# twice154/ofa-for-super-resolution

Hardware: AMD Instinct MI355X
Metric: sr_training_images_per_sec_4x_64to256 (higher is better)
Workload: dtype bf16; 1 GPU; OFA-SR S4 supernet 4x progressive shrinking (elastic kernel {3,5,7}, e=6, d=4, pd=2), LR 64x64 -> HR 256x256, fwd+bwd+Adam, train-mode BN; kernel_transform_mode=1, compat_reference_indexing=True, parallelism=dp1, per_gpu_batch=16, global_batch=16, grad_allreduce_bytes=0, launch=eager

## Files before the change

### include/ofasr.h

```cpp
#ifndef OFASR_H
#define OFASR_H

#include <stddef.h>
#include <stdint.h>

#ifdef __cplusplus
extern "C" {
#endif

#define OFASR_VERSION 303

typedef enum {
    OFASR_OK = 0,
    OFASR_ERR_INVALID_ARG = -1,
    OFASR_ERR_UNSUPPORTED = -2,
    OFASR_ERR_WORKSPACE = -3,
    OFASR_ERR_LAUNCH = -4
} ofasr_status;

typedef enum { OFASR_F32 = 0, OFASR_F16 = 1, OFASR_BF16 = 2 } ofasr_dtype;

int ofasr_version(void);
const char* ofasr_last_error_string(void);
const char* ofasr_status_string(int status);
// ... 151 lines not shown
                               const float* running_var, double eps, int64_t Cin, int64_t Cout, int K, int dtype,
                               void* operands, size_t operand_bytes, void* stream);
int ofasr_conv2d_infer_run(const void* x, void* y, int64_t N, int64_t Cin, int64_t Cout, int64_t H, int64_t W, int K,
                           int dtype, int act, const void* operands, size_t operand_bytes, void* stream);
int ofasr_conv2d_fwd(const void* x, const float* w, void* y, int64_t N, int64_t Cin, int64_t Cout, int64_t H, int64_t W,
                     int K, int dtype, void* workspace, size_t workspace_bytes, void* stream);
int ofasr_conv2d_dgrad(const void* dy, const float* w, void* dx, int64_t N, int64_t Cin, int64_t Cout, int64_t H,
                       int64_t W, int K, int dtype, void* workspace, size_t workspace_bytes, void* stream);
size_t ofasr_conv2d_wgrad_workspace(int64_t N, int64_t Cin, int64_t Cout, int64_t H, int64_t W, int K);
int ofasr_conv2d_wgrad(const void* dy, const void* x, float* dw, int64_t N, int64_t Cin, int64_t Cout, int64_t H,
                       int64_t W, int K, int dtype, void* workspace, size_t workspace_bytes, void* stream);

size_t ofasr_conv2d_f32_workspace(int64_t Cin, int64_t Cout, int K, int dgrad);
int ofasr_conv2d_f32_fwd(const void* x, const float* w, void* y, int64_t N, int64_t Cin, int64_t Cout, int64_t H, int64_t W,
                         int K, void* workspace, size_t workspace_bytes, void* stream);
int ofasr_conv2d_f32_dgrad(const void* dy, const float* w, void* dx, int64_t N, int64_t Cin, int64_t Cout, int64_t H,
                           int64_t W, int K, void* workspace, size_t workspace_bytes, void* stream);
size_t ofasr_conv2d_f32_wgrad_workspace(int64_t N, int64_t Cin, int64_t Cout, int64_t H, int64_t W, int K);
int ofasr_conv2d_f32_wgrad(const void* dy, const void* x, float* dw, int64_t N, int64_t Cin, int64_t Cout, int64_t H,
                           int64_t W, int K, void* workspace, size_t workspace_bytes, void* stream);

size_t ofasr_bicubic_resize_u8_workspace(int64_t planes, int64_t in_h, int64_t in_w, int64_t out_h, int64_t out_w);
int ofasr_bicubic_resize_u8(const void* src, void* dst, int64_t planes, int64_t in_h, int64_t in_w, int64_t out_h,
                            int64_t out_w, void* workspace, size_t workspace_bytes, void* stream);

int ofasr_tile_gather_u8(const void* img, int64_t H, int64_t W, const int64_t* origins, int64_t n, int64_t h, int64_t w,
                         void* out, int dtype, void* stream);
int ofasr_tile_scatter_u8(const void* src, int64_t n, int64_t sh, int64_t sw, int dtype, const int64_t* table, void* img,
                          int64_t OH, int64_t OW, int64_t max_eh, int64_t max_ew, void* stream);

int ofasr_debug_mbfused_tile(int width);
int ofasr_debug_mbfused_split(int enable);
int ofasr_debug_mbconv_bn_bwd_stat(int enable);
long long ofasr_debug_launch_count(const char* substr);
void ofasr_debug_reset_launch_counts(void);
const char* ofasr_debug_launch_table(void);
int ofasr_profile_enable(int on);
const char* ofasr_profile_read(void);

#ifdef __cplusplus
}
#endif
#endif
```

### ofa-for-super-resolution_amd/_C.py

```python
import ctypes
import os
import subprocess

import torch

_HERE = os.path.dirname(os.path.abspath(__file__))
LIB_PATH = os.environ.get("OFASR_LIB_PATH") or os.path.join(_HERE, "csrc", "libofasr_hip.so")

F32, F16, BF16 = 0, 1, 2

_lib = None

_c_i64 = ctypes.c_int64
_c_int = ctypes.c_int
_c_vp = ctypes.c_void_p
_c_sz = ctypes.c_size_t

SIGNATURES = {
    "ofasr_version": (_c_int, []),
    "ofasr_last_error_string": (ctypes.c_char_p, []),
    "ofasr_status_string": (ctypes.c_char_p, [_c_int]),
    "ofasr_pixel_shuffle": (_c_int, [_c_vp, _c_vp, _c_i64, _c_i64, _c_i64, _c_i64, _c_int, _c_int, _c_vp]),
    "ofasr_pixel_unshuffle": (_c_int, [_c_vp, _c_vp, _c_i64, _c_i64, _c_i64, _c_i64, _c_int, _c_int, _c_vp]),
    "ofasr_ktransform_fwd": (_c_int, [_c_vp, ctypes.POINTER(_c_int), _c_int, ctypes.POINTER(_c_vp), _c_int,
# ... 57 lines not shown
    "ofasr_mbconv_stat_floats": (_c_sz, [_c_vp]),
    "ofasr_mbconv_fwd": (_c_int, [_c_vp, _c_vp, _c_vp, _c_vp, _c_vp, _c_sz, _c_vp]),
    "ofasr_mbconv_bwd": (_c_int, [_c_vp, _c_vp, _c_vp, _c_vp, _c_vp, _c_vp, _c_vp, _c_vp, _c_vp, _c_sz, _c_vp]),
    "ofasr_mbstack_fwd": (_c_int, [_c_vp, _c_int, _c_vp, _c_vp]),
    "ofasr_mbstack_bwd": (_c_int, [_c_vp, _c_int, _c_vp, _c_vp, _c_vp]),
    "ofasr_mbconv_defer_join": (_c_int, [_c_int]),
    "ofasr_mbconv_join": (_c_int, [_c_vp]),
    "ofasr_side_stream": (_c_vp, []),
    "ofasr_bicubic_resize_u8_workspace": (_c_sz, [_c_i64, _c_i64, _c_i64, _c_i64, _c_i64]),
    "ofasr_bicubic_resize_u8": (_c_int, [_c_vp, _c_vp, _c_i64, _c_i64, _c_i64, _c_i64, _c_i64, _c_vp, _c_sz, _c_vp]),
    "ofasr_mbconv_infer_supported": (_c_int, [_c_vp]),
    "ofasr_mbconv_infer_workspace": (_c_sz, [_c_vp]),
    "ofasr_mbconv_infer": (_c_int, [_c_vp, _c_vp, _c_vp, _c_vp, _c_sz, _c_vp]),
    "ofasr_mbconv_infer_operand_bytes": (_c_sz, [_c_vp]),
    "ofasr_mbconv_infer_scratch_bytes": (_c_sz, [_c_vp]),
    "ofasr_mbconv_infer_prepare": (_c_int, [_c_vp, _c_vp, _c_sz, _c_vp]),
    "ofasr_mbconv_infer_run": (_c_int, [_c_vp, _c_vp, _c_vp, _c_vp, _c_sz, _c_vp, _c_sz, _c_vp]),
    "ofasr_mbconv_infer_f32_supported": (_c_int, [_c_vp]),
    "ofasr_mbconv_infer_f32_operand_bytes": (_c_sz, [_c_vp]),
    "ofasr_mbconv_infer_f32_scratch_bytes": (_c_sz, [_c_vp]),
    "ofasr_mbconv_infer_f32_prepare": (_c_int, [_c_vp, _c_vp, _c_sz, _c_vp]),
    "ofasr_mbconv_infer_f32_run": (_c_int, [_c_vp, _c_vp, _c_vp, _c_vp, _c_sz, _c_vp, _c_sz, _c_vp]),
    "ofasr_mbconv_recal_f32_supported": (_c_int, [_c_vp]),
    "ofasr_mbconv_recal_f32_workspace": (_c_sz, [_c_vp]),
    "ofasr_mbconv_recal_f32": (_c_int, [_c_vp, _c_vp, _c_vp, _c_vp, _c_vp, _c_vp, _c_vp, _c_sz, _c_vp]),
    "ofasr_bn_recal_accumulate": (_c_int, [_c_vp, _c_i64, _c_i64, ctypes.c_double, ctypes.c_double, _c_vp, _c_vp,
                                           ctypes.c_double, _c_vp, _c_vp, _c_vp]),
    "ofasr_tile_gather_u8": (_c_int, [_c_vp, _c_i64, _c_i64, _c_vp, _c_i64, _c_i64, _c_i64, _c_vp, _c_int, _c_vp]),
    "ofasr_tile_scatter_u8": (_c_int, [_c_vp, _c_i64, _c_i64, _c_i64, _c_int, _c_vp, _c_vp, _c_i64, _c_i64, _c_i64, _c_i64,
                                       _c_vp]),
    "ofasr_debug_mbfused_tile": (_c_int, [_c_int]),
    "ofasr_debug_mbfused_split": (_c_int, [_c_int]),
    "ofasr_debug_mbconv_bn_bwd_stat": (_c_int, [_c_int]),
    "ofasr_debug_launch_count": (ctypes.c_longlong, [ctypes.c_char_p]),
    "ofasr_debug_reset_launch_counts": (None, []),
    "ofasr_debug_launch_table": (ctypes.c_char_p, []),
    "ofasr_profile_enable": (_c_int, [_c_int]),
    "ofasr_profile_read": (ctypes.c_char_p, []),
}


def launch_count(substr=""):
    return int(lib().ofasr_debug_launch_count(substr.encode()))


def reset_launch_counts():
    lib().ofasr_debug_reset_launch_counts()


def launch_table():
    out = {}
    for line in lib().ofasr_debug_launch_table().decode().splitlines():
        n, name = line.split("\t", 1)
        if int(n):
            out[name] = int(n)
    return out


def profile_read():
    out = {}
    for line in lib().ofasr_profile_read().decode().splitlines():
        name, n, us, by, fl = line.rsplit("\t", 4)
        out[name] = {"launches": float(n), "total_us": float(us), "bytes": float(by), "flops": float(fl)}
    return out


# ... 57 lines not shown
```

### ofa-for-super-resolution_amd/csrc/mbconv.hip

```cpp
#include "ofasr_common.h"

#include <atomic>
#include <mutex>
#include <vector>

namespace ofasr {

static size_t align_up(size_t v, size_t a) { return (v + a - 1) / a * a; }
static bool bn_fold_enabled() {
    static const bool on = [] { const char* e = getenv("OFASR_MBCONV_BN_BWD_FOLD"); return !(e && e[0] == '0'); }();
    return on;
}
static thread_local int t_skip_kt = 0;
static std::atomic<int> g_bn_bwd_stat{[] { const char* e = getenv("OFASR_MBCONV_BN_BWD_STAT"); return (e && e[0] == '1') ? 1 : 0; }()};

struct MbSizes {
    size_t es;
    size_t mid_elems;
    size_t out_elems;
    size_t ws_bn;
    size_t ws_bn_bwd;
    size_t ws_dw;
    size_t ws_pw;
    size_t ws_kt;
    size_t scratch;
    size_t stat_a;
    size_t side;
    size_t df_bytes;
    size_t coef_off;
    size_t total;
};

static MbSizes mb_sizes(const ofasr_mbconv_desc* d) {
    MbSizes s;
    const int64_t HW = d->H * d->W;
    s.es = d->dtype == OFASR_F32 ? 4 : 2;
    s.mid_elems = (size_t)(d->N * d->mid * HW);
    s.out_elems = (size_t)(d->N * d->Cout * HW);
    const int64_t cbig = d->mid > d->Cout ? d->mid : d->Cout;
    s.ws_bn = align_up(ofasr_bn_workspace(d->N, cbig), 256);
    s.ws_bn_bwd = align_up(ofasr_bn_act_bwd_workspace(d->N, cbig), 256);
    s.ws_dw = align_up(ofasr_dwconv_wgrad_workspace(d->N, d->mid, d->H, d->W, d->K), 256);
    size_t pw1 = ofasr_pwconv_wgrad_workspace(d->N, d->Cin, d->mid, HW);
    size_t pw2 = ofasr_pwconv_wgrad_workspace(d->N, d->mid, d->Cout, HW);
    s.ws_pw = align_up(pw1 > pw2 ? pw1 : pw2, 256);
    s.ws_kt = align_up(ofasr_ktransform_bwd_workspace(d->ks, d->chain_len - 1, d->mid), 256);
    s.scratch = s.ws_bn > s.ws_bn_bwd ? s.ws_bn : s.ws_bn_bwd;
    {
        const size_t u1 = (size_t)pwconv_stat_units(d->N, d->Cin, HW) * (size_t)d->mid;
        const size_t u2 = (size_t)dwconv_stat_units(d->N, d->H, d->W, d->K, d->dtype) * (size_t)d->mid;
        const size_t u3 = (size_t)pwconv_stat_units(d->N, d->mid, HW) * (size_t)d->Cout;
        s.stat_a = align_up((u1 > u3 ? u1 : u3) * sizeof(float2), 256);
        const size_t ws_stat = s.stat_a + align_up(u2 * sizeof(float2), 256);
        if (ws_stat > s.scratch) s.scratch = ws_stat;
    }
    s.side = s.ws_dw > s.ws_pw ? s.ws_dw : s.ws_pw;
    s.df_bytes = align_up((size_t)(d->mid * d->K * d->K) * sizeof(float), 256);
    s.coef_off = s.scratch + s.side + s.df_bytes + s.ws_kt + 256;
    s.total = s.coef_off + align_up((size_t)(4 * d->mid) * sizeof(float), 256);
    return s;
}

static int check_desc(const char* name, const ofasr_mbconv_desc* d) {
    OFASR_REQUIRE(d != nullptr, OFASR_ERR_INVALID_ARG, "%s: null descriptor", name);
    OFASR_REQUIRE(d->N > 0 && d->Cin > 0 && d->mid > 0 && d->Cout > 0 && d->H > 0 && d->W > 0, OFASR_ERR_INVALID_ARG,
                  "%s: bad shape", name);
    OFASR_REQUIRE(d->chain_len >= 1 && d->chain_len <= 4, OFASR_ERR_INVALID_ARG, "%s: bad kernel chain", name);
    OFASR_REQUIRE(d->ks[d->chain_len - 1] == d->K, OFASR_ERR_INVALID_ARG, "%s: chain does not end at K", name);
    OFASR_REQUIRE(d->w1 && d->w2 && d->wdw_max, OFASR_ERR_INVALID_ARG, "%s: null weight", name);
    OFASR_REQUIRE(!d->residual || d->Cin == d->Cout, OFASR_ERR_INVALID_ARG, "%s: residual needs Cin == Cout", name);
    for (int i = 0; i < 3; ++i)
        OFASR_REQUIRE(d->gamma[i] && d->beta[i] && d->running_mean[i] && d->running_var[i], OFASR_ERR_INVALID_ARG,
                      "%s: null BN tensor %d", name, i);
    return OFASR_OK;
}

__global__ void bump_counters_kernel(int64_t* a, int64_t* b, int64_t* c) {
    if (threadIdx.x == 0) {
        if (a) *a += 1;
        if (b) *b += 1;
        if (c) *c += 1;
    }
}

struct PendingSide {
    const char *t0, *t1, *w0, *w1;
    hipEvent_t done;
};
constexpr size_t MAX_PENDING = 64;
struct SideStream {
    bool ready = false, enabled = true, defer = false;
    hipStream_t s = nullptr;
// ... 375 lines not shown
        if (e1 == hipSuccess) e1 = hipStreamWaitEvent(ss.s, ss.fork[i], 0);
        OFASR_REQUIRE(e1 == hipSuccess, OFASR_ERR_LAUNCH, "%s: stream fork failed: %s", name, hipGetErrorString(e1));
        return OFASR_OK;
    };
    const bool fused = lay.fused;
    if (fused)
        OFASR_REQUIRE((reinterpret_cast<uintptr_t>(tmp_buf) & 15) == 0, OFASR_ERR_UNSUPPORTED,
                      "%s: tmp_buf must be 16-byte aligned (the forward pass did not materialise the activations)", name);
    rc = fork(0);
    if (rc) return rc;
    if (split_fill && !prezeroed) {
        const hipError_t ef = fill(0, 3, (hipStream_t)sst);
        OFASR_REQUIRE(ef == hipSuccess, OFASR_ERR_LAUNCH, "%s: memset failed: %s", name, hipGetErrorString(ef));
    }
    if (fused)
        rc = pwconv_wgrad_xf(t3, y2, g->dw2, d->ldw2, d->N, d->mid, d->Cout, HW, d->dtype,
                             xf_of(stat_buf, 1, d->mid, d->Cout), side_ws, s.side, sst);
    else
        rc = ofasr_pwconv_wgrad(t3, a2, g->dw2, d->ldw2, d->N, d->mid, d->Cout, HW, d->dtype, side_ws, s.side, sst);
    if (rc) return rc;
    StatView s2 = stat_view(sb, 1, d->mid, d->Cout);
    StatView s1 = stat_view(sb, 0, d->mid, d->Cout);
    const bool bn_fold = bn_fold_enabled();
    float* coef = reinterpret_cast<float*>((char*)workspace + s.coef_off);
    void* tC = t + (2 * s.mid_elems + (size_t)d->N * d->Cout * HW) * s.es;
    const bool wg_bx = fused && bn_fold_enabled() &&
                       dwconv_wgrad_bx_supported(tA, y1, y2, d->N, d->mid, d->H, d->W, d->K, d->dtype);
    BwdXf bx2{y2, s2.mean, s2.scale, s2.shift, coef, coef + d->mid, wg_bx ? nullptr : tC};
    static const bool wg1_env = [] { const char* e = getenv("OFASR_MBCONV_WG1_BX"); return e && e[0] == '1'; }();
    const bool wg1_bx = fused && bn_fold && wg1_env &&
                        pwconv_wgrad_bx_supported(tB, y1, x, d->Cin, d->mid, HW, d->dtype);
    BwdXf bx1{y1, s1.mean, s1.scale, s1.shift, coef + 2 * d->mid, coef + 3 * d->mid,
              wg1_bx ? nullptr : (wg_bx ? tC : tA)};
    static const bool coef_fold = [] { const char* e = getenv("OFASR_MBCONV_BN_COEF_FOLD"); return !(e && e[0] == '0'); }();
    auto arm_fold = [&](BwdXf& bx, int P, const StatView& sv, int which) {
        bx.fold_partial = (const double*)workspace;
        bx.fold_P = P;
        bx.fold_C = (int)d->mid;
        bx.fold_training = d->bn_training[which];
        bx.fold_M = (double)d->N * (double)HW;
        bx.fold_invstd = sv.invstd;
        bx.fold_dgamma = g->dgamma[which];
        bx.fold_dbeta = g->dbeta[which];
        bx.coef_ka = const_cast<float*>(bx.ka);
        bx.coef_kbi = const_cast<float*>(bx.kbi);
    };
    const bool bxp = fused && bn_fold && dwconv_xf_supported(tA, tB, d->H, d->W, d->K, d->dtype) &&
                     (reinterpret_cast<uintptr_t>(tC) & 15) == 0 &&
                     pwconv_dgrad_bx_supported(tB, y1, dx, d->residual ? dout : nullptr, d->w1, d->ldw1, d->Cin, d->mid, HW,
                                               d->dtype);
    const bool bn_stat = g_bn_bwd_stat.load(std::memory_order_relaxed) != 0;
    const int P2b = pwconv_stat_units(d->N, d->Cout, HW);
    const bool st2 = bxp && bn_stat && pwconv_dgrad_bstat_supported(t3, y2, tA, d->w2, d->ldw2, d->mid, d->Cout, HW, d->dtype) &&
                     (size_t)P2b * (size_t)d->mid * sizeof(float2) <= s.stat_a;
    if (st2) {
        rc = pwconv_dgrad_bstat(t3, d->w2, d->ldw2, tA, d->N, d->mid, d->Cout, HW, d->dtype,
                                BwdStatOut{y2, s2.mean, s2.scale, s2.shift, (float2*)workspace, P2b}, stream);
        if (rc) return rc;
        rc = bn_bwd_coef_cp((const float2*)workspace, P2b, d->mid, (double)d->N * (double)HW, d->bn_training[1], s2.scale,
                            s2.invstd, g->dgamma[1], g->dbeta[1], coef, coef + d->mid, stream);
    } else {
        rc = ofasr_pwconv_dgrad(t3, d->w2, d->ldw2, tA, d->N, d->mid, d->Cout, HW, d->dtype, stream);
    }
    if (rc) return rc;
    if (bxp) {
        if (!st2 && coef_fold) {
// ... 5 lines not shown
        } else if (!st2) {
            rc = bn_bwd_reduce_coef(tA, y2, s2.scale, s2.shift, s2.mean, s2.invstd, g->dgamma[1], g->dbeta[1], coef,
                                    coef + d->mid, d->N, d->mid, HW, 1, d->bn_training[1], d->dtype, workspace, s.scratch,
                                    stream);
            if (rc) return rc;
        }
        rc = dwconv_dgrad_bx(tA, f, tB, d->N, d->mid, d->H, d->W, d->K, d->dtype, bx2, stream);
        if (rc) return rc;
        rc = fork(1);
        if (rc) return rc;
        if (wg_bx)
            rc = dwconv_wgrad_xf_bx(tA, y1, dfp, d->N, d->mid, d->H, d->W, d->K, d->dtype, xf_of(stat_buf, 0, d->mid, d->Cout),
                                    BwdXf{y2, s2.mean, s2.scale, s2.shift, coef, coef + d->mid, nullptr}, sst);
        else
            rc = dwconv_wgrad_xf(tC, y1, dfp, d->N, d->mid, d->H, d->W, d->K, d->dtype, xf_of(stat_buf, 0, d->mid, d->Cout),
                                 side_ws, s.side, sst);
        if (rc) return rc;
        rc = (t_skip_kt & 2) ? OFASR_OK
                             : ofasr_ktransform_bwd(d->wdw_max, d->ks, d->chain_len - 1, d->mats, d->transform, dfp, g->dwdw_max,
                                                    g->dmats, d->mid, kt_ws, s.ws_kt + 256, sst);
        if (rc) return rc;
        if (coef_fold) {
            int P1 = 0;
            rc = bn_bwd_reduce_only(tB, y1, s1.scale, s1.shift, s1.mean, s1.invstd, d->N, d->mid, HW, 1, d->dtype, workspace,
                                    s.scratch, &P1, stream);
            if (rc) return rc;
            arm_fold(bx1, P1, s1, 0);
        } else {
            rc = bn_bwd_reduce_coef(tB, y1, s1.scale, s1.shift, s1.mean, s1.invstd, g->dgamma[0], g->dbeta[0], coef + 2 * d->mid,
                                    coef + 3 * d->mid, d->N, d->mid, HW, 1, d->bn_training[0], d->dtype, workspace, s.scratch,
                                    stream);
        }
        if (rc) return rc;
        rc = pwconv_dgrad_add_bx(tB, d->w1, d->ldw1, dx, d->residual ? dout : nullptr, d->N, d->Cin, d->mid, HW, d->dtype, bx1,
                                 stream);
        if (rc) return rc;
        rc = fork(2);
        if (rc) return rc;
        if (wg1_bx)
            rc = pwconv_wgrad_bx(tB, x, g->dw1, d->ldw1, d->N, d->Cin, d->mid, HW, d->dtype,
                                 BwdXf{y1, s1.mean, s1.scale, s1.shift, coef + 2 * d->mid, coef + 3 * d->mid, nullptr}, side_ws,
                                 s.side, sst);
        else
            rc = ofasr_pwconv_wgrad(wg_bx ? tC : tA, x, g->dw1, d->ldw1, d->N, d->Cin, d->mid, HW, d->dtype, side_ws, s.side, sst);
        if (rc) return rc;
    } else {
    rc = ofasr_bn_act_bwd(tA, y2, nullptr, tA, nullptr, s2.scale, s2.shift, s2.mean, s2.invstd, g->dgamma[1],
                          g->dbeta[1], d->N, d->mid, HW, 1, d->bn_training[1], d->dtype, workspace, s.scratch, stream);
    if (rc) return rc;
    rc = fork(1);
    if (rc) return rc;
    if (fused)
        rc = dwconv_wgrad_xf(tA, y1, dfp, d->N, d->mid, d->H, d->W, d->K, d->dtype, xf_of(stat_buf, 0, d->mid, d->Cout),
                             side_ws, s.side, sst);
    else
        rc = ofasr_dwconv_wgrad(tA, a1, dfp, d->N, d->mid, d->H, d->W, d->K, d->dtype, side_ws, s.side, sst);
    if (rc) return rc;
    rc = (t_skip_kt & 2) ? OFASR_OK
                         : ofasr_ktransform_bwd(d->wdw_max, d->ks, d->chain_len - 1, d->mats, d->transform, dfp, g->dwdw_max,
                                                g->dmats, d->mid, kt_ws, s.ws_kt + 256, sst);
    if (rc) return rc;
    rc = ofasr_dwconv_dgrad(tA, f, tB, d->N, d->mid, d->H, d->W, d->K, d->dtype, stream);
    if (rc) return rc;
    rc = ofasr_bn_act_bwd(tB, y1, nullptr, tB, nullptr, s1.scale, s1.shift, s1.mean, s1.invstd, g->dgamma[0],
                          g->dbeta[0], d->N, d->mid, HW, 1, d->bn_training[0], d->dtype, workspace, s.scratch, stream);
    if (rc) return rc;
    rc = fork(2);
    if (rc) return rc;
    rc = ofasr_pwconv_wgrad(tB, x, g->dw1, d->ldw1, d->N, d->Cin, d->mid, HW, d->dtype, side_ws, s.side, sst);
    if (rc) return rc;
    if (d->residual)
        rc = pwconv_dgrad_add(tB, d->w1, d->ldw1, dx, dout, d->N, d->Cin, d->mid, HW, d->dtype, stream);
    else
        rc = ofasr_pwconv_dgrad(tB, d->w1, d->ldw1, dx, d->N, d->Cin, d->mid, HW, d->dtype, stream);
    if (rc) return rc;
    }
    if (par) {
        std::lock_guard<std::mutex> lk(ss.mu);
// ... 139 lines not shown
                hipEvent_t ev = nullptr;
                if (hipEventCreateWithFlags(&ev, hipEventDisableTiming) != hipSuccess) {
                    (void)hipGetLastError();
                    return join_side_locked(ss, as_stream(stream), "ofasr_mbstack_bwd");
                }
                ss.pool.push_back(ev);
            }
            const hipError_t e3 = hipEventRecord(ss.pool[k], ss.s);
            OFASR_REQUIRE(e3 == hipSuccess, OFASR_ERR_LAUNCH, "ofasr_mbstack_bwd: event record failed: %s", hipGetErrorString(e3));
            const char *wlo = nullptr, *whi = nullptr;
            for (int i = 0; i < n; ++i) {
                const char* w0 = (const char*)items[i].workspace;
                wlo = (!wlo || w0 < wlo) ? w0 : wlo;
                whi = (!whi || w0 + items[i].workspace_bytes > whi) ? w0 + items[i].workspace_bytes : whi;
            }
            ss.pending.push_back(PendingSide{nullptr, nullptr, wlo, whi, ss.pool[k]});
        } else {
            rc = join_side_locked(ss, as_stream(stream), "ofasr_mbstack_bwd");
        }
    }
    return rc;
}

OFASR_EXPORT int ofasr_mbconv_bwd(const ofasr_mbconv_desc* d, const void* x, const void* act_buf, const float* stat_buf,
                                  const void* dout, void* dx, void* tmp_buf, const ofasr_mbconv_grads* g,
                                  void* workspace, size_t workspace_bytes, void* stream) {
    return mbconv_bwd_impl(d, x, act_buf, stat_buf, dout, dx, tmp_buf, g, workspace, workspace_bytes, stream, false);
}

OFASR_EXPORT int ofasr_debug_mbconv_bn_bwd_stat(int enable) {
    return g_bn_bwd_stat.exchange(enable ? 1 : 0, std::memory_order_relaxed);
}

OFASR_EXPORT int ofasr_mbconv_defer_join(int enable) {
    SideStream& ss = side_stream();
    std::lock_guard<std::mutex> lk(ss.mu);
    const int was = ss.defer ? 1 : 0;
    if (!enable && ss.defer && !ss.pending.empty()) {
        (void)hipStreamSynchronize(ss.s);
        ss.pending.clear();
    }
    ss.defer = ss.enabled && enable != 0;
    return was;
}

OFASR_EXPORT void* ofasr_side_stream(void) {
    SideStream& ss = side_stream();
    return ss.enabled ? (void*)ss.s : nullptr;
}

OFASR_EXPORT int ofasr_mbconv_join(void* stream) {
    SideStream& ss = side_stream();
    std::lock_guard<std::mutex> lk(ss.mu);
    if (ss.pending.empty()) return OFASR_OK;
    return join_side_locked(ss, as_stream(stream), "ofasr_mbconv_join");
}
```

### ofa-for-super-resolution_amd/csrc/ofasr_common.h

```cpp
#pragma once
#include <hip/hip_runtime.h>
#include <hip/hip_ext.h>
#include <tuple>
#include <utility>
#include <stdint.h>
#include <stdio.h>
#include "../../include/ofasr.h"

#define OFASR_EXPORT extern "C" __attribute__((visibility("default")))

namespace ofasr {

void set_error(const char* fmt, ...);

inline hipStream_t as_stream(void* s) { return reinterpret_cast<hipStream_t>(s); }

inline int check_launch(const char* what) {
    hipError_t e = hipGetLastError();
    if (e != hipSuccess) {
        set_error("%s: launch failed: %s", what, hipGetErrorString(e));
        return OFASR_ERR_LAUNCH;
    }
    return OFASR_OK;
}
// ... 288 lines not shown
bool conv_thin_wgrad_supported(int64_t Ct, int64_t Cw, int K, int64_t H, int64_t W, int dtype, const void* a, const void* b);
size_t conv_thin_wgrad_workspace(int64_t N, int64_t Ct, int64_t Cw, int64_t H, int64_t W, int K, int dtype);
int conv_thin_wgrad(const void* dy, const void* x, float* dw, int64_t N, int64_t Cin, int64_t Cout, int64_t H, int64_t W, int K,
                    int dtype, void* workspace, size_t workspace_bytes, void* stream);
bool conv_thin_in_supported(int64_t Ct, int64_t Cw, int K, int64_t W, int dtype, const void* x, const void* y);
int conv_thin_in_units(int64_t N, int64_t Ct, int64_t Cw, int64_t H, int64_t W, int dtype);
int conv_thin_in(const void* x, const float* w, void* y, int64_t N, int64_t Ct, int64_t Cw, int64_t H, int64_t W, int K,
                 int dtype, int dgrad, StatOut so, void* stream);

bool dwconv_xf_supported(const void* x, const void* y, int64_t H, int64_t W, int K, int dtype);
bool dwconv_stat_supported(const void* x, const void* y, int64_t H, int64_t W, int K, int dtype);
int dwconv_fwd_stat(const void* x, const float* f, void* y, int64_t N, int64_t C, int64_t H, int64_t W, int K, int dtype,
                    StatOut so, void* stream);
int dwconv_fwd_xf(const void* x, const float* f, void* y, int64_t N, int64_t C, int64_t H, int64_t W, int K, int dtype,
                  InputXf xf, void* stream, StatOut so = StatOut{nullptr, 0}, BnFold fold = BnFold{});
int dwconv_wgrad_xf(const void* dy, const void* x, float* df, int64_t N, int64_t C, int64_t H, int64_t W, int K,
                    int dtype, InputXf xf, void* workspace, size_t workspace_bytes, void* stream);
bool dwconv_wgrad_bx_supported(const void* da, const void* x, const void* y, int64_t N, int64_t C, int64_t H, int64_t W,
                               int K, int dtype);
int dwconv_wgrad_xf_bx(const void* da, const void* x, float* df, int64_t N, int64_t C, int64_t H, int64_t W, int K,
                       int dtype, InputXf xf, BwdXf bx, void* stream);
int dwconv_dgrad_bx(const void* da, const float* f, void* dx, int64_t N, int64_t C, int64_t H, int64_t W, int K,
                    int dtype, BwdXf bx, void* stream);
int bn_finalize_bump(const void* workspace, int64_t n_partials, int64_t C, double count, const float* gamma,
                     const float* beta, float* running_mean, float* running_var, double momentum, double eps,
                     int training, float* mean, float* invstd, float* scale, float* shift, int64_t* k0, int64_t* k1,
                     int64_t* k2, void* stream);
int pwconv_dgrad_add(const void* dy, const float* w, int64_t ldw, void* dx, const void* addend, int64_t N, int64_t Cin,
                     int64_t Cout, int64_t HW, int dtype, void* stream);
bool pwconv_dgrad_bx_supported(const void* da, const void* y, const void* dx, const void* addend, const float* w,
                               int64_t ldw, int64_t Cin, int64_t Cout, int64_t HW, int dtype);
int pwconv_dgrad_add_bx(const void* da, const float* w, int64_t ldw, void* dx, const void* addend, int64_t N, int64_t Cin,
                        int64_t Cout, int64_t HW, int dtype, BwdXf bx, void* stream);
bool pwconv_xf_supported(const void* x, const void* y, int64_t HW, int dtype);
int pwconv_fwd_xf(const void* x, const float* w, int64_t ldw, void* y, int64_t N, int64_t Cin, int64_t Cout, int64_t HW,
                  int dtype, InputXf xf, void* stream, StatOut so = StatOut{nullptr, 0});
bool pwconv_fold_supported(const void* x, const void* y, const float* w, int64_t ldw, int64_t Cin, int64_t HW, int dtype);
int pwconv_fwd_fold(const void* x, const float* w, int64_t ldw, void* y, int64_t N, int64_t Cin, int64_t Cout,
                    int64_t HW, int dtype, BnFold fold, void* stream, StatOut so = StatOut{nullptr, 0});
int pwconv_fwd_stat(const void* x, const float* w, int64_t ldw, void* y, int64_t N, int64_t Cin, int64_t Cout,
                    int64_t HW, int dtype, StatOut so, void* stream);
bool pwconv_wgrad_bx_supported(const void* da, const void* y, const void* x, int64_t Cin, int64_t Cout, int64_t HW, int dtype);
int pwconv_wgrad_bx(const void* da, const void* x, float* dw, int64_t ldw, int64_t N, int64_t Cin, int64_t Cout, int64_t HW,
                    int dtype, BwdXf bx, void* workspace, size_t workspace_bytes, void* stream);
int pwconv_wgrad_xf(const void* dy, const void* x, float* dw, int64_t ldw, int64_t N, int64_t Cin, int64_t Cout,
                    int64_t HW, int dtype, InputXf xf, void* workspace, size_t workspace_bytes, void* stream);

}
```

### ofa-for-super-resolution_amd/csrc/pwconv.hip

```cpp
#include <stdlib.h>
#include "ofasr_common.h"

namespace ofasr {

typedef __attribute__((ext_vector_type(16))) float f32x16;
typedef __attribute__((ext_vector_type(8))) __bf16 bf16x8;
typedef __attribute__((ext_vector_type(8))) _Float16 f16x8;
typedef __attribute__((ext_vector_type(4))) short s16x4;
typedef __attribute__((ext_vector_type(8))) short s16x8;
typedef __attribute__((address_space(3))) s16x4 lds_s16x4;

constexpr int PW_THREADS = 256;
constexpr int PW_TILE = 128;
constexpr int XROW16 = 320;
constexpr int XROW32 = 512;
constexpr int WROW16 = 128;
constexpr int WROW32 = 256;

template <typename T> struct Mma16;
template <> struct Mma16<bf16_t> {
    static __device__ __forceinline__ f32x16 run(s16x8 a, s16x8 b, f32x16 c) {
        return __builtin_amdgcn_mfma_f32_32x32x16_bf16(__builtin_bit_cast(bf16x8, a), __builtin_bit_cast(bf16x8, b),
                                                       c, 0, 0, 0);
    }
// ... 1092 lines not shown
        T* yw = yn + (long long)(32 * cb) * HW + px;
        if (addend) {
            const T* aw = addend + ((long long)n * wv.M + m_base + 32 * cb) * HW + px;
            uint32_t ar[16];
#pragma unroll
            for (int reg = 0; reg < 16; ++reg)
                ar[reg] = *reinterpret_cast<const uint32_t*>(aw + (long long)acc_row(reg, h) * HW);
#pragma unroll
            for (int reg = 0; reg < 16; ++reg) {
                T lo, hi;
                lo.v = (uint16_t)(ar[reg] & 0xffffu);
                hi.v = (uint16_t)(ar[reg] >> 16);
                acc[0][reg] += to_float(lo);
                acc[1][reg] += to_float(hi);
            }
        }
#pragma unroll
        for (int reg = 0; reg < 16; ++reg)
            *reinterpret_cast<uint32_t*>(yw + (long long)acc_row(reg, h) * HW) = pack2<T>(acc[0][reg], acc[1][reg]);
        if (so.partial) stat_epilogue<T, 2>(acc, px, HW, c, h, 32 * cb, mloc, m_base, so, 2 * tile + hh);
        return;
    }
#pragma unroll
    for (int reg = 0; reg < 16; ++reg) {
        const int r = 32 * cb + acc_row(reg, h);
        if (r < mloc) {
            float v[2] = {acc[0][reg], acc[1][reg]};
            if (addend)
                add_px<T, 2, true>(addend + ((long long)n * wv.M + m_base + r) * HW, p0 + 64 * hh + 2 * c, HW, v);
            store_px<T, 2, true>(yn + (long long)r * HW, p0 + 64 * hh + 2 * c, HW, v);
        }
    }
    if (so.partial) stat_epilogue<T, 2>(acc, p0 + 64 * hh + 2 * c, HW, c, h, 32 * cb, mloc, m_base, so, 2 * tile + hh);
}

template <typename T, bool ALIGNED>
__device__ __forceinline__ void stage_rows64(char* Lt, const T* __restrict__ base, int rows_total, int r0, int HW,
                                             int p0) {
    const int tid = threadIdx.x;
    if constexpr (Elem<T>::is16) {
        if (ALIGNED) {
#pragma unroll
            for (int it = 0; it < 2; ++it) {
                const int q = tid + it * PW_THREADS;
                const int r = q >> 3, ch = q & 7;
                const int px = p0 + 8 * ch;
                uint4 v = make_uint4(0, 0, 0, 0);
                if (r0 + r < rows_total && px < HW)
                    v = *reinterpret_cast<const uint4*>(base + (long long)(r0 + r) * HW + px);
                *reinterpret_cast<uint4*>(Lt + wtile_chunk_off<T>(r, ch)) = v;
            }
        } else {
            for (int e = tid; e < 64 * 64; e += PW_THREADS) {
                const int r = e >> 6, k = e & 63;
                uint16_t v = 0;
                if (r0 + r < rows_total && p0 + k < HW)
                    v = reinterpret_cast<const uint16_t*>(base)[(long long)(r0 + r) * HW + p0 + k];
                *reinterpret_cast<uint16_t*>(Lt + wtile_off<T>(r, k)) = v;
            }
        }
    } else {
        if (ALIGNED) {
#pragma unroll
            for (int it = 0; it < 4; ++it) {
                const int q = tid + it * PW_THREADS;
                const int r = q >> 4, ch = q & 15;
// ... 640 lines not shown
template <typename T>
static int launch_dgrad_bx(const char* name, const void* da, WView wv, void* dx, const void* addend, int64_t N, int64_t HW,
                           BwdXf bx, hipStream_t st) {
    const int tiles_per_img = (int)cdiv(HW, PW_TILE);
    const int64_t total64 = N * tiles_per_img;
    OFASR_REQUIRE(total64 <= INT32_MAX, OFASR_ERR_UNSUPPORTED, "%s: too many pixel tiles", name);
    {
        const double px = (double)N * (double)HW, es = (double)sizeof(T);
        prof_note(es * px * (2.0 * wv.K + wv.M + (addend ? wv.M : 0)) + 4.0 * wv.K * wv.M, 2.0 * px * wv.K * wv.M);
    }
    dim3 grid((unsigned)total64, (unsigned)cdiv(wv.M, 64));
    OFASR_LAUNCH((pw_fanin_pipe_kernel<T, false, true, true>), grid, dim3(PW_THREADS), 0, st, (const T*)da, wv, (T*)dx,
                 (int)HW, tiles_per_img, (int)cdiv(wv.K, 64), InputXf{}, (const T*)addend, StatOut{nullptr, 0}, BnFold{}, bx);
    return check_launch(name);
}

int pwconv_dgrad_add_bx(const void* da, const float* w, int64_t ldw, void* dx, const void* addend, int64_t N, int64_t Cin,
                        int64_t Cout, int64_t HW, int dtype, BwdXf bx, void* stream) {
    const char* name = "pwconv_dgrad_add_bx";
    int rc = check_pw_args(name, da, w, dx, ldw, N, Cin, Cout, HW, dtype);
    if (rc) return rc;
    OFASR_REQUIRE(bx.y && bx.mean && bx.scale && bx.shift &&
                      ((bx.ka && bx.kbi) || (bx.fold_partial && bx.fold_invstd && bx.fold_P > 0 && bx.fold_C == Cout)),
                  OFASR_ERR_INVALID_ARG, "%s: null transform", name);
    OFASR_REQUIRE(pwconv_dgrad_bx_supported(da, bx.y, dx, addend, w, ldw, Cin, Cout, HW, dtype), OFASR_ERR_UNSUPPORTED,
                  "%s: needs the pipelined fan-in kernel (aligned 16-bit tensors, 64 < Cout <= %d)", name, FOLD_KMAX);
    if (N * HW == 0) return OFASR_OK;
    WView wv{w, 1, ldw, (int)Cin, (int)Cout};
    hipStream_t st = as_stream(stream);
    if (dtype == OFASR_F16) return launch_dgrad_bx<f16_t>(name, da, wv, dx, addend, N, HW, bx, st);
    return launch_dgrad_bx<bf16_t>(name, da, wv, dx, addend, N, HW, bx, st);
}

bool pwconv_xf_supported(const void* x, const void* y, int64_t HW, int dtype) {
    return (dtype == OFASR_F16 || dtype == OFASR_BF16) && aligned_for(x, y, HW, true);
}

bool pwconv_dgrad_bstat_supported(const void* dy, const void* y, const void* dx, const float* w, int64_t ldw, int64_t Cin,
                                  int64_t Cout, int64_t HW, int dtype) {
    const bool wvec = (reinterpret_cast<uintptr_t>(w) & 15) == 0 && (ldw % 4) == 0;
    return (dtype == OFASR_F16 || dtype == OFASR_BF16) && aligned_for(dy, dx, HW, true) &&
           (reinterpret_cast<uintptr_t>(y) & 15) == 0 && wvec && Cout == 64 && (Cin == 2 * FO_ROWS || Cin == 3 * FO_ROWS) &&
           HW % PW_TILE == 0;
}

template <typename T>
static int launch_dgrad_bstat(const void* dy, WView wv, void* dx, int64_t N, int64_t HW, BwdStatOut bs, hipStream_t st) {
    const int tiles_per_img = (int)(HW / PW_TILE);
    const int total_tiles = (int)(N * tiles_per_img);
    const double px = (double)N * (double)HW;
    prof_note(2.0 * px * (wv.K + 2.0 * wv.M) + 4.0 * wv.K * wv.M, 2.0 * px * wv.K * wv.M);
    if (wv.M == 3 * FO_ROWS)
        OFASR_LAUNCH((pw_fanout_slabs_kernel<T, 3, 2>), dim3((unsigned)total_tiles), dim3(PW_THREADS), 0, st, (const T*)dy, wv,
                     (T*)dx, (int)HW, tiles_per_img, StatOut{nullptr, 0}, bs);
    else
        OFASR_LAUNCH((pw_fanout_slabs_kernel<T, 2, 2>), dim3((unsigned)total_tiles), dim3(PW_THREADS), 0, st, (const T*)dy, wv,
                     (T*)dx, (int)HW, tiles_per_img, StatOut{nullptr, 0}, bs);
    return check_launch("pwconv_dgrad_bstat");
}

int pwconv_dgrad_bstat(const void* dy, const float* w, int64_t ldw, void* dx, int64_t N, int64_t Cin, int64_t Cout,
                       int64_t HW, int dtype, BwdStatOut bs, void* stream) {
    const char* name = "pwconv_dgrad_bstat";
    int rc = check_pw_args(name, dy, w, dx, ldw, N, Cin, Cout, HW, dtype);
    if (rc) return rc;
    OFASR_REQUIRE(bs.y && bs.mean && bs.scale && bs.shift && bs.partial, OFASR_ERR_INVALID_ARG, "%s: null pointer", name);
// ... 160 lines not shown
```

Baseline: 2713 images/s.

## Fuse expand-conv weight gradient into the BN-backward dgrad fan-in kernel

Adds a kernel that, while computing the first pointwise conv's input gradient with the BN backward transform applied on load, also accumulates the weight gradient from the same transformed tiles against the block input, writing per-block fp32 slabs. A separate reduction then sums the slabs into dw1 on the side stream. This removes the separate wgrad pass that re-read the transformed gradient and input from memory. In exchange it adds shared-memory pressure, slab workspace and an extra reduction launch. It is enabled by default when the shape allows and there are at least 256 pixel-pair tiles.

```diff
diff --git a/include/ofasr.h b/include/ofasr.h
--- a/include/ofasr.h
+++ b/include/ofasr.h
@@ -207,6 +207,7 @@
 int ofasr_debug_mbfused_tile(int width);
 int ofasr_debug_mbfused_split(int enable);
 int ofasr_debug_mbconv_bn_bwd_stat(int enable);
+int ofasr_debug_mbconv_wg1_fused(int enable);
 long long ofasr_debug_launch_count(const char* substr);
 void ofasr_debug_reset_launch_counts(void);
 const char* ofasr_debug_launch_table(void);
diff --git a/ofa-for-super-resolution_amd/_C.py b/ofa-for-super-resolution_amd/_C.py
--- a/ofa-for-super-resolution_amd/_C.py
+++ b/ofa-for-super-resolution_amd/_C.py
@@ -113,6 +113,7 @@
     "ofasr_debug_mbfused_tile": (_c_int, [_c_int]),
     "ofasr_debug_mbfused_split": (_c_int, [_c_int]),
     "ofasr_debug_mbconv_bn_bwd_stat": (_c_int, [_c_int]),
+    "ofasr_debug_mbconv_wg1_fused": (_c_int, [_c_int]),
     "ofasr_debug_launch_count": (ctypes.c_longlong, [ctypes.c_char_p]),
     "ofasr_debug_reset_launch_counts": (None, []),
     "ofasr_debug_launch_table": (ctypes.c_char_p, []),
diff --git a/ofa-for-super-resolution_amd/csrc/mbconv.hip b/ofa-for-super-resolution_amd/csrc/mbconv.hip
--- a/ofa-for-super-resolution_amd/csrc/mbconv.hip
+++ b/ofa-for-super-resolution_amd/csrc/mbconv.hip
@@ -13,6 +13,7 @@
 }
 static thread_local int t_skip_kt = 0;
 static std::atomic<int> g_bn_bwd_stat{[] { const char* e = getenv("OFASR_MBCONV_BN_BWD_STAT"); return (e && e[0] == '1') ? 1 : 0; }()};
+static std::atomic<int> g_wg1_fused{[] { const char* e = getenv("OFASR_MBCONV_WG1_FUSED"); return (e && (e[0] == '0' || e[0] == '1')) ? e[0] - '0' : -1; }()};
 
 struct MbSizes {
     size_t es;
@@ -28,6 +29,8 @@
     size_t side;
     size_t df_bytes;
     size_t coef_off;
+    size_t wg1_off;
+    size_t wg1_bytes;
     size_t total;
 };
 
@@ -57,7 +60,10 @@
     s.side = s.ws_dw > s.ws_pw ? s.ws_dw : s.ws_pw;
     s.df_bytes = align_up((size_t)(d->mid * d->K * d->K) * sizeof(float), 256);
     s.coef_off = s.scratch + s.side + s.df_bytes + s.ws_kt + 256;
-    s.total = s.coef_off + align_up((size_t)(4 * d->mid) * sizeof(float), 256);
+    s.wg1_off = s.coef_off + align_up((size_t)(4 * d->mid) * sizeof(float), 256);
+    const bool wg1_shape = d->dtype != OFASR_F32 && d->Cin == 64 && d->mid % 64 == 0 && d->mid > 64 && d->mid <= 384 && HW % 256 == 0;
+    s.wg1_bytes = wg1_shape ? align_up(pwconv_dgrad_bx_wg_workspace(d->N, d->Cin, d->mid, HW), 256) : 0;
+    s.total = s.wg1_off + s.wg1_bytes;
     return s;
 }
 
@@ -499,6 +505,8 @@
                         pwconv_wgrad_bx_supported(tB, y1, x, d->Cin, d->mid, HW, d->dtype);
     BwdXf bx1{y1, s1.mean, s1.scale, s1.shift, coef + 2 * d->mid, coef + 3 * d->mid,
               wg1_bx ? nullptr : (wg_bx ? tC : tA)};
+    const int wg1_sw = g_wg1_fused.load(std::memory_order_relaxed);
+    const bool wg1_fused_on = wg1_sw > 0 || (wg1_sw < 0 && d->N * (HW / 256) >= 256);
     static const bool coef_fold = [] { const char* e = getenv("OFASR_MBCONV_BN_COEF_FOLD"); return !(e && e[0] == '0'); }();
     auto arm_fold = [&](BwdXf& bx, int P, const StatView& sv, int which) {
         bx.fold_partial = (const double*)workspace;
@@ -570,6 +578,21 @@
                                     stream);
         }
         if (rc) return rc;
+        const bool wg1_fused = wg1_fused_on && s.wg1_bytes > 0 &&
+                               pwconv_dgrad_bx_wg_supported(tB, y1, dx, d->residual ? dout : nullptr, d->w1, d->ldw1, x, d->Cin,
+                                                            d->mid, HW, d->dtype);
+        if (wg1_fused) {
+            char* slabs = (char*)workspace + s.wg1_off;
+            int nslabs = 0;
+            bx1.dy_out = nullptr;
+            rc = pwconv_dgrad_add_bx_wg(tB, d->w1, d->ldw1, dx, d->residual ? dout : nullptr, x, d->N, d->Cin, d->mid, HW,
+                                        d->dtype, bx1, slabs, s.wg1_bytes, &nslabs, stream);
+            if (rc) return rc;
+            rc = fork(2);
+            if (rc) return rc;
+            rc = pwconv_wg_slab_reduce(slabs, nslabs, g->dw1, d->ldw1, d->Cin, d->mid, sst);
+            if (rc) return rc;
+        } else {
         rc = pwconv_dgrad_add_bx(tB, d->w1, d->ldw1, dx, d->residual ? dout : nullptr, d->N, d->Cin, d->mid, HW, d->dtype, bx1,
                                  stream);
         if (rc) return rc;
@@ -582,6 +605,7 @@
         else
             rc = ofasr_pwconv_wgrad(wg_bx ? tC : tA, x, g->dw1, d->ldw1, d->N, d->Cin, d->mid, HW, d->dtype, side_ws, s.side, sst);
         if (rc) return rc;
+        }
     } else {
     rc = ofasr_bn_act_bwd(tA, y2, nullptr, tA, nullptr, s2.scale, s2.shift, s2.mean, s2.invstd, g->dgamma[1],
                           g->dbeta[1], d->N, d->mid, HW, 1, d->bn_training[1], d->dtype, workspace, s.scratch, stream);
@@ -787,6 +811,10 @@
     return g_bn_bwd_stat.exchange(enable ? 1 : 0, std::memory_order_relaxed);
 }
 
+OFASR_EXPORT int ofasr_debug_mbconv_wg1_fused(int enable) {
+    return g_wg1_fused.exchange(enable < 0 ? -1 : (enable ? 1 : 0), std::memory_order_relaxed);
+}
+
 OFASR_EXPORT int ofasr_mbconv_defer_join(int enable) {
     SideStream& ss = side_stream();
     std::lock_guard<std::mutex> lk(ss.mu);
diff --git a/ofa-for-super-resolution_amd/csrc/ofasr_common.h b/ofa-for-super-resolution_amd/csrc/ofasr_common.h
--- a/ofa-for-super-resolution_amd/csrc/ofasr_common.h
+++ b/ofa-for-super-resolution_amd/csrc/ofasr_common.h
@@ -344,6 +344,13 @@
                                int64_t ldw, int64_t Cin, int64_t Cout, int64_t HW, int dtype);
 int pwconv_dgrad_add_bx(const void* da, const float* w, int64_t ldw, void* dx, const void* addend, int64_t N, int64_t Cin,
                         int64_t Cout, int64_t HW, int dtype, BwdXf bx, void* stream);
+bool pwconv_dgrad_bx_wg_supported(const void* da, const void* y, const void* dx, const void* addend, const float* w,
+                                  int64_t ldw, const void* x, int64_t Cin, int64_t Cout, int64_t HW, int dtype);
+size_t pwconv_dgrad_bx_wg_workspace(int64_t N, int64_t Cin, int64_t Cout, int64_t HW);
+int pwconv_dgrad_add_bx_wg(const void* da, const float* w, int64_t ldw, void* dx, const void* addend, const void* x,
+                           int64_t N, int64_t Cin, int64_t Cout, int64_t HW, int dtype, BwdXf bx, void* slabs,
+                           size_t slab_bytes, int* nslabs, void* stream);
+int pwconv_wg_slab_reduce(const void* slabs, int nslabs, float* dw, int64_t ldw, int64_t Cin, int64_t Cout, void* stream);
 bool pwconv_xf_supported(const void* x, const void* y, int64_t HW, int dtype);
 int pwconv_fwd_xf(const void* x, const float* w, int64_t ldw, void* y, int64_t N, int64_t Cin, int64_t Cout, int64_t HW,
                   int dtype, InputXf xf, void* stream, StatOut so = StatOut{nullptr, 0});
diff --git a/ofa-for-super-resolution_amd/csrc/pwconv.hip b/ofa-for-super-resolution_amd/csrc/pwconv.hip
--- a/ofa-for-super-resolution_amd/csrc/pwconv.hip
+++ b/ofa-for-super-resolution_amd/csrc/pwconv.hip
@@ -1148,6 +1148,196 @@
         }
     }
     if (so.partial) stat_epilogue<T, 2>(acc, p0 + 64 * hh + 2 * c, HW, c, h, 32 * cb, mloc, m_base, so, 2 * tile + hh);
+}
+
+constexpr int WGF_THREADS = 512;
+constexpr int WGF_XT_ROW = 256;
+__device__ __forceinline__ int wgf_xt_off(int row, int chunk) { return row * WGF_XT_ROW + ((chunk ^ (row & 15)) << 4); }
+
+template <typename T, int KC>
+__global__ void __launch_bounds__(WGF_THREADS) pw_fanin_wg_kernel(const T* __restrict__ da, const float* __restrict__ w,
+                                                                  long long ldw, T* __restrict__ dx,
+                                                                  const T* __restrict__ xin, float* __restrict__ part,
+                                                                  int HW, int pairs_per_img, int npairs,
+                                                                  const T* __restrict__ addend, BwdXf bx) {
+    constexpr int K = 64 * KC;
+    constexpr int M = 64;
+    __shared__ __attribute__((aligned(16))) char Ws[64 * WROW16];
+    __shared__ __attribute__((aligned(16))) char Xs[2][64 * XROW16];
+    __shared__ __attribute__((aligned(16))) char Xn[2][64 * WGF_XT_ROW];
+    __shared__ __attribute__((aligned(16))) char Xt[2][64 * WGF_XT_ROW];
+    __shared__ float bxt[5 * K];
+    const int tid = threadIdx.x;
+    for (int ch = tid; ch < K; ch += WGF_THREADS) {
+        const float mu = bx.mean[ch], sc = bx.scale[ch];
+        bxt[ch] = mu;
+        bxt[K + ch] = sc;
+        bxt[2 * K + ch] = fmaf(mu, sc, bx.shift[ch]);
+        if (bx.fold_partial) {
+            float ka, kbi;
+            bwdxf_fold(bx, ch, sc, blockIdx.x == 0, ka, kbi);
+            bxt[3 * K + ch] = ka;
+            bxt[4 * K + ch] = kbi;
+        } else {
+            bxt[3 * K + ch] = bx.ka[ch];
+            bxt[4 * K + ch] = bx.kbi[ch];
+        }
+    }
+    __syncthreads();
+    const int lane = lane_id();
+    const int wave = __builtin_amdgcn_readfirstlane((int)(threadIdx.x >> 6));
+    const int half = wave >> 2;
+    const int t = tid & 255;
+    const int c = lane & 31, h = lane >> 5;
+    const int cb = wave & 1, hh = (wave >> 1) & 1;
+    char* Xh = Xs[half];
+    uint32_t xoff[4], woff[2];
+#pragma unroll
+    for (int it = 0; it < 4; ++it) {
+        const int q = t + it * 256;
+        xoff[it] = (uint32_t)(q >> 4) * (uint32_t)HW + 8u * (q & 15);
+    }
+#pragma unroll
+    for (int it = 0; it < 2; ++it) {
+        const int q = tid + it * WGF_THREADS;
+        woff[it] = (uint32_t)(q >> 4) * (uint32_t)ldw + 4u * (q & 15);
+    }
+    constexpr int NOWN = (KC + 1) / 2;
+    f32x16 dwa[NOWN];
+#pragma unroll
+    for (int o = 0; o < NOWN; ++o) dwa[o] = zero16();
+    const int row = 32 * cb + c;
+
+    const int pair_lo = (int)((long long)blockIdx.x * npairs / gridDim.x);
+    const int pair_hi = (int)((long long)(blockIdx.x + 1) * npairs / gridDim.x);
+    for (int pair = pair_lo; pair < pair_hi; ++pair) {
+        const int n = pair / pairs_per_img;
+        const int p0 = (pair - n * pairs_per_img) * (2 * PW_TILE) + PW_TILE * half;
+        const T* dan = da + (long long)n * K * HW + p0;
+        const T* y1n = reinterpret_cast<const T*>(bx.y) + (long long)n * K * HW + p0;
+#pragma unroll
+        for (int it = 0; it < 4; ++it) asm volatile("" : "+v"(xoff[it]));
+#pragma unroll
+        for (int it = 0; it < 2; ++it) asm volatile("" : "+v"(woff[it]));
+        uint4 xr[4], yr[4], xt[4];
+        float4 wr[2];
+        auto load_chunk = [&](int kc) {
+#pragma unroll
+            for (int it = 0; it < 4; ++it) asm volatile("" : "+v"(xoff[it]));
+#pragma unroll
+            for (int it = 0; it < 2; ++it) asm volatile("" : "+v"(woff[it]));
+            const float* wk = w + (long long)(64 * kc) * ldw;
+            const T* xk = dan + (long long)(64 * kc) * HW;
+            const T* yk = y1n + (long long)(64 * kc) * HW;
+#pragma unroll
+            for (int it = 0; it < 2; ++it) wr[it] = *reinterpret_cast<const float4*>(wk + woff[it]);
+#pragma unroll
+            for (int it = 0; it < 4; ++it) {
+                xr[it] = *reinterpret_cast<const uint4*>(xk + xoff[it]);
+                yr[it] = *reinterpret_cast<const uint4*>(yk + xoff[it]);
+            }
+        };
+        auto store_chunk = [&](int kc) {
+            asm volatile("" ::: "memory");
+#pragma unroll
+            for (int it = 0; it < 2; ++it) {
+                const int q = tid + it * WGF_THREADS;
+                const int k = q >> 4, r = 4 * (q & 15);
+                lds_store_w<T>(Ws, wtile_off<T>(r, k), wr[it].x);
+                lds_store_w<T>(Ws, wtile_off<T>(r + 1, k), wr[it].y);
+                lds_store_w<T>(Ws, wtile_off<T>(r + 2, k), wr[it].z);
+                lds_store_w<T>(Ws, wtile_off<T>(r + 3, k), wr[it].w);
+            }
+#pragma unroll
+            for (int it = 0; it < 4; ++it) {
+                const int q = t + it * 256;
+                const int k = q >> 4, m = q & 15;
+                const int ch = 64 * kc + k;
+                const uint4 v = bx_apply8<T>(xr[it], yr[it], bxt[ch], bxt[K + ch], bxt[2 * K + ch], bxt[3 * K + ch], bxt[4 * K + ch]);
+                *reinterpret_cast<uint4*>(Xn[half] + wgf_xt_off(k, m)) = v;
+                char* rowp = Xh + k * XROW16;
+                const int base = 64 * (m >> 3) + 4 * (m & 7);
+                *reinterpret_cast<uint2*>(rowp + base * 2) =
+                    make_uint2((v.x & 0xffffu) | (v.y << 16), (v.z & 0xffffu) | (v.w << 16));
+                *reinterpret_cast<uint2*>(rowp + (base + 32) * 2) =
+                    make_uint2((v.x >> 16) | (v.y & 0xffff0000u), (v.z >> 16) | (v.w & 0xffff0000u));
+            }
+        };
+        {
+            const T* xn = xin + (long long)n * M * HW + p0;
+#pragma unroll
+            for (int it = 0; it < 4; ++it) xt[it] = *reinterpret_cast<const uint4*>(xn + xoff[it]);
+        }
+        load_chunk(0);
+        if (pair != pair_lo) __syncthreads();
+#pragma unroll
+        for (int it = 0; it < 4; ++it) {
+            const int q = t + it * 256;
+            *reinterpret_cast<uint4*>(Xt[half] + wgf_xt_off(q >> 4, q & 15)) = xt[it];
+        }
+        f32x16 acc[2];
+        acc[0] = zero16();
+        acc[1] = zero16();
+        auto dw_round = [&](f32x16& d) {
+#pragma unroll
+            for (int tl = 0; tl < 2; ++tl) {
+#pragma unroll
+                for (int qj = 0; qj < 8; ++qj) {
+                    if ((qj & 3) == 0) __builtin_amdgcn_sched_barrier(0);
+                    const int chunk = 8 * (qj >> 2) + 4 * h + (qj & 3);
+                    const s16x8 a = *reinterpret_cast<const s16x8*>(Xn[tl] + wgf_xt_off(32 * cb + c, chunk));
+                    const s16x8 b = *reinterpret_cast<const s16x8*>(Xt[tl] + wgf_xt_off(32 * hh + c, chunk));
+                    d = Mma16<T>::run(a, b, d);
+                }
+            }
+        };
+#pragma unroll
+        for (int kc = 0; kc < KC; ++kc) {
+            __builtin_amdgcn_sched_barrier(0);
+            if (kc) __syncthreads();
+            store_chunk(kc);
+            __syncthreads();
+            if (kc + 1 < KC) load_chunk(kc + 1);
+#pragma unroll
+            for (int s = 0; s < 4; ++s) {
+                const s16x8 af = *reinterpret_cast<const s16x8*>(Ws + wtile_chunk_off<T>(row, 2 * s + h));
+                const s16x8 b0 = read_b_frag16(Xh, 64 * hh, s, lane);
+                const s16x8 b1 = read_b_frag16(Xh, 64 * hh + 32, s, lane);
+                acc[0] = Mma16<T>::run(af, b0, acc[0]);
+                acc[1] = Mma16<T>::run(af, b1, acc[1]);
+            }
+            if ((kc & 1) == half) dw_round(dwa[kc >> 1]);
+        }
+        const int px = 64 * hh + 2 * c;
+        T* yw = dx + ((long long)n * M + 32 * cb) * HW + p0 + px;
+        if (addend) {
+            const T* aw = addend + ((long long)n * M + 32 * cb) * HW + p0 + px;
+            uint32_t ar[16];
+#pragma unroll
+            for (int reg = 0; reg < 16; ++reg)
+                ar[reg] = *reinterpret_cast<const uint32_t*>(aw + (long long)acc_row(reg, h) * HW);
+#pragma unroll
+            for (int reg = 0; reg < 16; ++reg) {
+                T lo, hi;
+                lo.v = (uint16_t)(ar[reg] & 0xffffu);
+                hi.v = (uint16_t)(ar[reg] >> 16);
+                acc[0][reg] += to_float(lo);
+                acc[1][reg] += to_float(hi);
+            }
+        }
+#pragma unroll
+        for (int reg = 0; reg < 16; ++reg)
+            *reinterpret_cast<uint32_t*>(yw + (long long)acc_row(reg, h) * HW) = pack2<T>(acc[0][reg], acc[1][reg]);
+    }
+    float* slab = part + (long long)blockIdx.x * K * M;
+#pragma unroll
+    for (int o = 0; o < NOWN; ++o) {
+        const int kc = 2 * o + half;
+        if (kc < KC) {
+#pragma unroll
+            for (int reg = 0; reg < 16; ++reg) slab[(64 * kc + 32 * cb + acc_row(reg, h)) * M + 32 * hh + c] = dwa[o][reg];
+        }
+    }
 }
 
 template <typename T, bool ALIGNED>
@@ -1854,6 +2044,81 @@
     return launch_dgrad_bx<bf16_t>(name, da, wv, dx, addend, N, HW, bx, st);
 }
 
+constexpr int WGF_KC_MAX = 6;
+static int wgf_blocks(int64_t N, int64_t HW) {
+    static const int blocks = [] { const char* e = getenv("OFASR_PW_WGRAD_BLOCKS"); const int v = e ? atoi(e) : 0; return v > 0 ? v : 256; }();
+    const int64_t pairs = N * (HW / (2 * PW_TILE));
+    return (int)(pairs < blocks ? pairs : blocks);
+}
+
+bool pwconv_dgrad_bx_wg_supported(const void* da, const void* y, const void* dx, const void* addend, const float* w,
+                                  int64_t ldw, const void* x, int64_t Cin, int64_t Cout, int64_t HW, int dtype) {
+    return pwconv_dgrad_bx_supported(da, y, dx, addend, w, ldw, Cin, Cout, HW, dtype) &&
+           (reinterpret_cast<uintptr_t>(x) & 15) == 0 && Cin == 64 && Cout % 64 == 0 && Cout <= 64 * WGF_KC_MAX &&
+           HW % (2 * PW_TILE) == 0;
+}
+
+size_t pwconv_dgrad_bx_wg_workspace(int64_t N, int64_t Cin, int64_t Cout, int64_t HW) {
+    if (N <= 0 || HW < 2 * PW_TILE) return 0;
+    return (size_t)wgf_blocks(N, HW) * (size_t)Cin * (size_t)Cout * sizeof(float);
+}
+
+template <typename T, int KC>
+static void launch_dgrad_bx_wg(const void* da, const float* w, int64_t ldw, void* dx, const void* addend, const void* x,
+                               int64_t N, int64_t HW, BwdXf bx, float* slabs, int blocks, hipStream_t st) {
+    const int ppi = (int)(HW / (2 * PW_TILE));
+    OFASR_LAUNCH((pw_fanin_wg_kernel<T, KC>), dim3((unsigned)blocks), dim3(WGF_THREADS), 0, st, (const T*)da, w,
+                 (long long)ldw, (T*)dx, (const T*)x, slabs, (int)HW, ppi, (int)(N * ppi), (const T*)addend, bx);
+}
+
+int pwconv_dgrad_add_bx_wg(const void* da, const float* w, int64_t ldw, void* dx, const void* addend, const void* x,
+                           int64_t N, int64_t Cin, int64_t Cout, int64_t HW, int dtype, BwdXf bx, void* slabs,
+                           size_t slab_bytes, int* nslabs, void* stream) {
+    const char* name = "pwconv_dgrad_add_bx_wg";
+    int rc = check_pw_args(name, da, w, dx, ldw, N, Cin, Cout, HW, dtype);
+    if (rc) return rc;
+    OFASR_REQUIRE(x && slabs && nslabs, OFASR_ERR_INVALID_ARG, "%s: null pointer", name);
+    OFASR_REQUIRE(bx.y && bx.mean && bx.scale && bx.shift &&
+                      ((bx.ka && bx.kbi) || (bx.fold_partial && bx.fold_invstd && bx.fold_P > 0 && bx.fold_C == Cout)),
+                  OFASR_ERR_INVALID_ARG, "%s: null transform", name);
+    OFASR_REQUIRE(bx.dy_out == nullptr, OFASR_ERR_INVALID_ARG, "%s: this kernel stores no dy", name);
+    OFASR_REQUIRE(N * HW > 0 && pwconv_dgrad_bx_wg_supported(da, bx.y, dx, addend, w, ldw, x, Cin, Cout, HW, dtype),
+                  OFASR_ERR_UNSUPPORTED, "%s: needs aligned 16-bit tensors, Cin = 64, Cout = 64 k <= %d, HW %% 256 == 0", name,
+                  64 * WGF_KC_MAX);
+    const size_t need = pwconv_dgrad_bx_wg_workspace(N, Cin, Cout, HW);
+    OFASR_REQUIRE(slab_bytes >= need, OFASR_ERR_WORKSPACE, "%s: workspace %zu B < required %zu B", name, slab_bytes, need);
+    OFASR_REQUIRE(N * (HW / (2 * PW_TILE)) <= INT32_MAX, OFASR_ERR_UNSUPPORTED, "%s: too many pixel tiles", name);
+    const int blocks = wgf_blocks(N, HW);
+    *nslabs = blocks;
+    hipStream_t st = as_stream(stream);
+    {
+        const double px = (double)N * (double)HW, es = 2.0;
+        prof_note(es * px * (2.0 * Cout + 2.0 * Cin + (addend ? Cin : 0)) + 4.0 * Cout * Cin + 4.0 * blocks * (double)Cout * Cin,
+                  4.0 * px * Cout * Cin);
+    }
+#define OFASR_WGF(KC_)                                                                                                 \
+    case KC_:                                                                                                          \
+        if (dtype == OFASR_F16) launch_dgrad_bx_wg<f16_t, KC_>(da, w, ldw, dx, addend, x, N, HW, bx, (float*)slabs, blocks, st); \
+        else launch_dgrad_bx_wg<bf16_t, KC_>(da, w, ldw, dx, addend, x, N, HW, bx, (float*)slabs, blocks, st);        \
+        break;
+    switch ((int)(Cout / 64)) {
+        OFASR_WGF(2) OFASR_WGF(3) OFASR_WGF(4) OFASR_WGF(5) OFASR_WGF(6)
+        default: set_error("%s: Cout = %lld outside the instantiated kernels", name, (long long)Cout); return OFASR_ERR_UNSUPPORTED;
+    }
+#undef OFASR_WGF
+    return check_launch(name);
+}
+
+int pwconv_wg_slab_reduce(const void* slabs, int nslabs, float* dw, int64_t ldw, int64_t Cin, int64_t Cout, void* stream) {
+    const char* name = "pwconv_wg_slab_reduce";
+    OFASR_REQUIRE(slabs && dw && nslabs > 0 && ldw >= Cin, OFASR_ERR_INVALID_ARG, "%s: bad argument", name);
+    const long long tot = (long long)Cout * Cin;
+    prof_note(4.0 * (double)tot * (nslabs + 1.0), (double)tot * nslabs);
+    OFASR_LAUNCH(pw_wgrad_reduce_kernel, dim3((unsigned)cdiv(tot, 64)), dim3(64 * WR_ZL), 0, as_stream(stream),
+                 (const float*)slabs, dw, (int)Cout, (int)Cin, nslabs, (long long)ldw, 1LL);
+    return check_launch(name);
+}
+
 bool pwconv_xf_supported(const void* x, const void* y, int64_t HW, int dtype) {
     return (dtype == OFASR_F16 || dtype == OFASR_BF16) && aligned_for(x, y, HW, true);
 }
```

Measured after the change: 2769 images/s (median of 6 runs). 2.1% higher.
